# pangenome/povu

Hardware: AMD Instinct MI355X
Metric: edges/sec decomposed (flubble+PVST) (higher is better)
Workload: dtype u32

## Files before the change

### povu_amd/csrc/hip/common.hpp

```cpp
#pragma once
#include <hip/hip_runtime.h>

#include "forest_wire.hpp"

#include <algorithm>
#include <cstdint>
#include <cstdio>
#include <cstring>
#include <stdexcept>
#include <string>
#include <vector>

#define POVU_NIL 0xFFFFFFFFu

__device__ __forceinline__ uint4 load4_unaligned(const unsigned *__restrict__ p)
{
	typedef unsigned v4a __attribute__((ext_vector_type(4), aligned(4)));
	const v4a v = *reinterpret_cast<const v4a *>(p);
	return make_uint4(v.x, v.y, v.z, v.w);
}

#ifdef POVU_XCD_SWIZZLE
__device__ __forceinline__ unsigned povu_xcd_bid()
{
	const unsigned nwg = gridDim.x, q = nwg >> 3, r = nwg & 7u, x = blockIdx.x & 7u, i = blockIdx.x >> 3;
	return (x < r ? x * (q + 1) : r * (q + 1) + (x - r) * q) + i;
}
#define BIDX povu_xcd_bid()
#else
#define BIDX blockIdx.x
#endif

namespace povu_hip
{

struct HipError : std::runtime_error {
	using std::runtime_error::runtime_error;
};

#define HIP_CHECK(expr)                                                                          \
	do {                                                                                     \
		hipError_t e__ = (expr);                                                         \
		if (e__ != hipSuccess)                                                           \
			throw povu_hip::HipError(std::string(#expr) + ": " + hipGetErrorString(e__) + " (" + \
						 __FILE__ + ":" + std::to_string(__LINE__) + ")");   \
	} while (0)

#define KLAUNCH(kernel, grid, block, shmem, stream, ...)                                          \
	do {                                                                                      \
		hipLaunchKernelGGL(kernel, grid, block, shmem, stream, __VA_ARGS__);              \
		HIP_CHECK(hipGetLastError());                                                     \
	} while (0)
static constexpr int TPB = 256;
static inline unsigned nblk(size_t n) { return (unsigned)((n + TPB - 1) / TPB); }
#define LAUNCH(k, n, s, ...)                                                                     \
	do {                                                                                     \
		if ((n) > 0) {                                                                   \
			hipLaunchKernelGGL(k, dim3(nblk(n)), dim3(TPB), 0, s, __VA_ARGS__);      \
			HIP_CHECK(hipGetLastError());                                            \
		}                                                                                \
	} while (0)

struct XferTally {
	uint64_t h2d = 0, d2h = 0;
};
inline XferTally &xfer_tally()
{
	static thread_local XferTally t;
	return t;
}
inline hipError_t copy_async(void *dst, const void *src, size_t n, hipMemcpyKind kind, hipStream_t s)
{
	if (kind == hipMemcpyHostToDevice)
		xfer_tally().h2d += n;
	else if (kind == hipMemcpyDeviceToHost)
		xfer_tally().d2h += n;
	return hipMemcpyAsync(dst, src, n, kind, s);
}
inline void count_kernel_d2h(size_t n) { xfer_tally().d2h += n; }

class Arena
{
public:
	~Arena() { release(); }
	void release()
	{
		if (base_)
			(void)hipFree(base_);
		base_ = nullptr;
		cap_ = 0;
		top_ = 0;
	}
	void reserve(size_t bytes, bool head_room = true)
	{
		if (bytes > cap_) {
			release();
			size_t want = head_room ? bytes + bytes / 8 + (1u << 20) : bytes + 4096;
			if (hipMalloc(&base_, want) != hipSuccess) {
				(void)hipGetLastError();
				base_ = nullptr;
				want = bytes + 4096;
				if (hipMalloc(&base_, want) != hipSuccess) {
// ... 401 lines not shown
```

### povu_amd/csrc/hip/tree_kernels.hip

```cpp
#include "tree_kernels.hpp"

#include <cstdlib>

#include <algorithm>
#include <type_traits>
#include <vector>

namespace povu_hip
{

#ifndef NIL
#define NIL POVU_NIL
#endif

static unsigned rank_bucket_bits(size_t n)
{
	if (const char *ev = getenv("POVU_HIP_RANK_BITS"))
		return (unsigned)std::min(6, std::max(2, atoi(ev)));
	(void)n;
	return 3u;
}
static constexpr uint32_t PK_END = 0x1FFFFFFFu, PK_STOP = 0x80000000u;
static constexpr uint32_t P0_END = 0x3FFFFFFFu, P0_W = 0x40000000u, P0_HEAD = 0x80000000u;
static constexpr uint32_t FT_NONE = 0x7FFFFFFFu, FT_HASH = 0x80000000u;
__device__ __forceinline__ uint32_t bucket_splitter(uint32_t q, unsigned b) { return (q << b) | ((q * 0x9E3779B1u) >> (32u - b)); }
__device__ __forceinline__ bool is_splitter(uint32_t i, unsigned b) { return bucket_splitter(i >> b, b) == i; }
__device__ __forceinline__ uint32_t rank_pack(uint32_t nx, uint32_t w, unsigned b)
{
	(void)b;
	return (nx == NIL ? P0_END : nx) | ((w & 1u) ? P0_W : 0u);
}
__device__ __forceinline__ bool rank_l0_stop(uint32_t nx, unsigned b) { return nx == P0_END || is_splitter(nx, b); }

__device__ __forceinline__ uint32_t find_link_slot(const uint32_t *__restrict__ loff, const uint32_t *__restrict__ lle, uint32_t w,
						   uint32_t le)
{
	uint32_t lo = loff[w], hi = loff[w + 1];
	const uint32_t l0 = lo;
	if (hi - lo > 8) {
		while (lo < hi) {
			const uint32_t mid = (lo + hi) >> 1;
			if ((lle[mid] & LLE_ID) < le)
				lo = mid + 1;
			else
				hi = mid;
		}
		return lo - l0 + 1;
	}
	for (uint32_t j = lo; j < hi; j++)
		if ((lle[j] & LLE_ID) == le)
			return j - l0 + 1;
	return 0;
}
__device__ __forceinline__ void store2_unaligned(uint32_t *p, uint32_t a, uint32_t b)
{
	typedef uint32_t v2a __attribute__((ext_vector_type(2), aligned(4)));
	v2a v;
	v.x = a;
	v.y = b;
	*reinterpret_cast<v2a *>(p) = v;
}
__device__ __forceinline__ void zero2(uint32_t *p) { store2_unaligned(p, 0u, 0u); }
__device__ __forceinline__ void zero2(uint8_t *p) { p[0] = p[1] = 0; }
__device__ __forceinline__ uint32_t arc_twin(const uint32_t *__restrict__ loff, const uint32_t *__restrict__ ladj,
					     const uint32_t *__restrict__ lle, uint32_t at)
{
	const uint32_t w = ladj[at];
	return loff[w] + find_link_slot(loff, lle, w, lle[at] & LLE_ID) - 1;
}
__device__ __forceinline__ ulonglong2 link_hash(uint32_t le)
{
	unsigned long long z = ((unsigned long long)le + 1ull) * 0x9E3779B97F4A7C15ull;
	z = (z ^ (z >> 30)) * 0xBF58476D1CE4E5B9ull;
	z = (z ^ (z >> 27)) * 0x94D049BB133111EBull;
	unsigned long long y = ((unsigned long long)le ^ 0x5851F42D4C957F2Dull) * 0xD6E8FEB86659FD93ull;
	y = (y ^ (y >> 33)) * 0xFF51AFD7ED558CCDull;
	y = (y ^ (y >> 33)) * 0xC4CEB9FE1A85EC53ull;
	return make_ulonglong2(z ^ (z >> 31), y ^ (y >> 33));
}
__device__ __forceinline__ ulonglong2 hx(const ulonglong2 a, const ulonglong2 b) { return make_ulonglong2(a.x ^ b.x, a.y ^ b.y); }
__device__ __forceinline__ bool hzero(const ulonglong2 a) { return (a.x | a.y) == 0ull; }
__device__ __forceinline__ bool heq(const ulonglong2 a, const ulonglong2 b) { return a.x == b.x && a.y == b.y; }
__global__ void k_tour_words(uint32_t nS, const uint32_t *__restrict__ loff, const uint32_t *__restrict__ ladj,
			     const uint32_t *__restrict__ lle, uint32_t *__restrict__ pk, unsigned b,
			     ulonglong2 *__restrict__ hside, uint32_t *__restrict__ ft)
{
	uint32_t S = BIDX * blockDim.x + threadIdx.x;
	if (S >= nS)
		return;
	const uint32_t lo = loff[S], hi = loff[S + 1];
	ulonglong2 h = make_ulonglong2(0ull, 0ull);
	uint32_t first = NIL;
	for (uint32_t at0 = lo; at0 < hi; at0 += 4) {
		const uint32_t rem = hi - at0;
		const uint4 lw4 = load4_unaligned(lle + at0), w4 = load4_unaligned(ladj + at0);
		const uint32_t lws[4] = {lw4.x, lw4.y, lw4.z, lw4.w}, ws[4] = {w4.x, w4.y, w4.z, w4.w};
		bool tree[4];
		uint2 o01[4];
		uint32_t se[4];
#pragma unroll
		for (uint32_t q = 0; q < 4; q++) {
			tree[q] = q < rem && (lws[q] & LLE_TREE);
			o01[q] = make_uint2(0u, 0u);
			se[q] = 0;
			if (tree[q]) {
				const uint32_t g2 = ws[q] & ~1u;
				o01[q] = *reinterpret_cast<const uint2 *>(loff + g2);
				se[q] = loff[g2 + 2];
			}
		}
		uint4 a[4];
#pragma unroll
		for (uint32_t q = 0; q < 4; q++) {
			a[q] = make_uint4(0u, 0u, 0u, 0u);
			if (tree[q] && se[q] - o01[q].x <= 8)
				a[q] = load4_unaligned(lle + o01[q].x);
		}
#pragma unroll
		for (uint32_t q = 0; q < 4; q++) {
			if (q >= rem)
				break;
			const uint32_t at = at0 + q, lw = lws[q], le = lw & LLE_ID;
			if (!tree[q]) {
				pk[at] = P0_END;
				h = hx(h, link_hash(le));
				continue;
			}
			if (first == NIL)
				first = at;
			const uint32_t w = ws[q], sb = o01[q].x;
			const uint32_t wl = (w & 1u) ? o01[q].y : sb, wh = (w & 1u) ? se[q] : o01[q].y;
			uint32_t nxt;
			if (se[q] - sb <= 8) {
				const uint32_t n = se[q] - sb, tl = wl - sb, th = wh - sb;
				uint4 c = make_uint4(0u, 0u, 0u, 0u);
				if (n > 4)
					c = load4_unaligned(lle + sb + 4);
				const uint32_t r[8] = {a[q].x, a[q].y, a[q].z, a[q].w, c.x, c.y, c.z, c.w};
				uint32_t tk = 0, first_tree = NIL, after = NIL;
#pragma unroll
				for (uint32_t k = 0; k < 8; k++)
					if (k >= tl && k < th && (r[k] & LLE_ID) == le)
						tk = k;
#pragma unroll
				for (uint32_t k = 0; k < 8; k++)
					if (k < n && (r[k] & LLE_TREE)) {
						if (first_tree == NIL)
							first_tree = k;
						if (k > tk && after == NIL)
							after = k;
					}
				nxt = sb + (after != NIL ? after : (first_tree < tk ? first_tree : tk));
			} else {
				const uint32_t t = wl + find_link_slot(loff, lle, w, le) - 1;
				nxt = t;
				for (uint32_t jj = t + 1; jj < se[q] && nxt == t; jj++)
					if (lle[jj] & LLE_TREE)
						nxt = jj;
				for (uint32_t jj = sb; jj < t && nxt == t; jj++)
					if (lle[jj] & LLE_TREE)
						nxt = jj;
			}
			pk[at] = rank_pack(nxt, 1u, b);
		}
	}
	const bool nz = !hzero(h);
	if (nz)
		hside[S] = h;
	ft[S] = (first == NIL ? FT_NONE : first) | (nz ? FT_HASH : 0u);
}
__device__ __forceinline__ uint32_t comp_root_side(const unsigned long long *start_key, const uint32_t *voff, uint32_t c)
{
	unsigned long long k = start_key[c];
	return k == ~0ull ? 2 * voff[c] : (uint32_t)(k & 0xFFFFFFFFu);
}
__global__ void k_tour_ends(uint32_t C, const uint32_t *__restrict__ voff, const unsigned long long *__restrict__ start_key,
			    const uint32_t *__restrict__ loff, const uint32_t *__restrict__ ladj, const uint32_t *__restrict__ lle,
			    uint32_t *__restrict__ pk, uint32_t *__restrict__ heads)
{
	uint32_t c = BIDX * blockDim.x + threadIdx.x;
	if (c >= C)
		return;
	const uint32_t r = comp_root_side(start_key, voff, c), sb = loff[r & ~1u], se = loff[(r & ~1u) + 2], mid = loff[r];
	uint32_t a_first = NIL, a_last = NIL;
	for (uint32_t j = mid; j < se; j++)
		if (lle[j] & LLE_TREE) {
			if (a_first == NIL)
				a_first = j;
			a_last = j;
		}
	for (uint32_t j = sb; j < mid; j++)
		if (lle[j] & LLE_TREE) {
			if (a_first == NIL)
				a_first = j;
			a_last = j;
		}
	heads[c] = a_first;
	if (a_first == NIL)
		return;
	pk[arc_twin(loff, ladj, lle, a_last)] = P0_END;
// ... 159 lines not shown
		return;
	uint32_t sa = ra[id], sb = TWO ? rb[id] : 0, p;
	do {
		p = nx_in[x];
		const uint32_t wa = a_io[x];
		a_io[x] = sa;
		sa -= wa;
		if (TWO) {
			const uint32_t wb = b_io[x];
			b_io[x] = sb;
			sb -= wb;
		}
		x = p & PK_END;
	} while (!(p & PK_STOP));
}
template <bool TWO>
__global__ void __launch_bounds__(1024) k_rank_top(uint32_t n, const uint32_t *__restrict__ nx_in, uint32_t *a_io, uint32_t *b_io)
{
	__shared__ uint32_t nx[RANK_TOP], sa[RANK_TOP], sb[TWO ? RANK_TOP : 1];
	for (uint32_t i = threadIdx.x; i < n; i += blockDim.x) {
		const uint32_t p = nx_in[i] & PK_END;
		nx[i] = p == PK_END ? NIL : p;
		sa[i] = a_io[i];
		if (TWO)
			sb[i] = b_io[i];
	}
	__syncthreads();
	constexpr int PER = RANK_TOP / 1024;
	for (uint32_t span = 1; span < n; span <<= 1) {
		uint32_t tn[PER], ta[PER], tb[PER];
#pragma unroll
		for (int k = 0; k < PER; k++) {
			const uint32_t i = threadIdx.x + k * 1024;
			tn[k] = NIL, ta[k] = 0, tb[k] = 0;
			if (i < n && nx[i] != NIL) {
				const uint32_t j = nx[i];
				tn[k] = nx[j];
				ta[k] = sa[j];
				if (TWO)
					tb[k] = sb[j];
			}
		}
		__syncthreads();
#pragma unroll
		for (int k = 0; k < PER; k++) {
			const uint32_t i = threadIdx.x + k * 1024;
			if (i < n && nx[i] != NIL) {
				nx[i] = tn[k];
				sa[i] += ta[k];
				if (TWO)
					sb[i] += tb[k];
			}
		}
		__syncthreads();
	}
	for (uint32_t i = threadIdx.x; i < n; i += blockDim.x) {
		a_io[i] = sa[i];
		if (TWO)
			b_io[i] = sb[i];
	}
}
__global__ void k_rank_unpack_next(uint32_t n, const uint32_t *__restrict__ nx_in, uint32_t *__restrict__ out)
{
	uint32_t i = BIDX * blockDim.x + threadIdx.x;
	if (i < n) {
		const uint32_t p = nx_in[i] & PK_END;
		out[i] = p == PK_END ? NIL : p;
	}
}

struct RankBufs {
	uint32_t *pk;
	uint32_t *heads;
	uint32_t *nx, *wa, *wb;
	uint32_t *tA, *tB, *tC;
};
static constexpr int RANK_MAX_LEVELS = 12;
static size_t rank_pool_words(size_t n, size_t nh) { return n / 2 + 4 * nh + 64; }

struct L0Ranks {
	const uint32_t *ra, *rb, *fin;
	uint32_t M;
};
__device__ __forceinline__ uint32_t rank_l0(const L0Ranks &R, uint2 rec)
{
	return (rec.x < R.M ? R.ra[rec.x] : 0u) - rec.y;
}
__device__ __forceinline__ uint32_t rank_l0_a(const L0Ranks &R, uint2 rec, bool fin)
{
	return fin ? rec.x : (rec.x < R.M ? R.ra[rec.x] : 0u) - (rec.y & REC_MAX);
}
__device__ __forceinline__ uint2 rank_l0_pair(const L0Ranks &R, uint2 rec, bool fin)
{
	if (fin)
		return rec;
	const bool in = rec.x < R.M;
	const uint32_t ra = in ? R.ra[rec.x] : 0u, rb = in ? R.rb[rec.x] : 0u, pa = rec.y & REC_MAX;
	return make_uint2(ra - pa, rb - pa + (rec.y >> 16));
}

template <bool TWO, bool EVT3 = false>
static L0Ranks list_rank_splitters(uint32_t n, unsigned b, uint2 *rec, uint32_t *ovf, uint32_t nh, RankBufs &rb, hipStream_t s)
{
	if (n >= P0_END)
		throw HipError("list ranking: more than 2^30 elements (graph too large for the packed walk)");
	RankLevelArgs lv[RANK_MAX_LEVELS];
	uint32_t *nxp[RANK_MAX_LEVELS + 1], *wap[RANK_MAX_LEVELS + 1], *wbp[RANK_MAX_LEVELS + 1];
	int levels = 0;
	size_t used = 0;
	const size_t pool = rank_pool_words(n, nh);
	nxp[0] = rb.pk, wap[0] = wbp[0] = nullptr;
	uint32_t cur_n = n, hbase = 0;
	for (;;) {
		RankLevelArgs &A = lv[levels];
		A.n = cur_n;
		A.m = (cur_n + (1u << b) - 1) >> b;
		A.hbase = hbase;
		A.M = A.m + nh;
		if (used + A.M > pool)
			throw HipError("list ranking: level pool exhausted (internal sizing bug)");
		nxp[levels + 1] = rb.nx + used, wap[levels + 1] = rb.wa + used, wbp[levels + 1] = rb.wb + used;
		used += A.M;
		levels++;
		hbase = A.m;
		const uint32_t next_n = A.M;
		if (next_n <= RANK_TOP || next_n > cur_n / 2 || levels == RANK_MAX_LEVELS) {
			cur_n = next_n;
			break;
		}
		cur_n = next_n;
	}
	if (TWO)
		HIP_CHECK(hipMemsetAsync(ovf, 0, 4, s));
	for (int L = 0; L < levels; L++) {
		const RankLevelArgs &A = lv[L];
		if (L == 0)
			LAUNCH((k_rank_up<true, TWO, EVT3>), A.M, s, A, b, nxp[0], nullptr, nullptr, rb.heads, nxp[1], wap[1], wbp[1], rec, ovf);
		else
			LAUNCH((k_rank_up<false, TWO>), A.M, s, A, b, nxp[L], wap[L], wbp[L], nullptr, nxp[L + 1], wap[L + 1], wbp[L + 1],
			       nullptr, nullptr);
	}
	const uint32_t nt = cur_n;
	if (nt <= RANK_TOP) {
		KLAUNCH((k_rank_top<TWO>), dim3(1), dim3(1024), 0, s, nt, nxp[levels], wap[levels], wbp[levels]);
	} else {
		LAUNCH(k_rank_unpack_next, nt, s, nt, nxp[levels], rb.tA);
		HIP_CHECK(copy_async(rb.tB, wap[levels], (size_t)nt * 4, hipMemcpyDeviceToDevice, s));
		if (TWO)
			HIP_CHECK(copy_async(rb.tC, wbp[levels], (size_t)nt * 4, hipMemcpyDeviceToDevice, s));
		uint32_t *nA = rb.tA, *nB = nxp[levels], *aA = rb.tB, *aB = wap[levels], *bA = rb.tC, *bB = wbp[levels];
		const int side = list_rank(nt, bits_for(nt) + 1, nA, nB, aA, aB, TWO ? bA : nullptr, TWO ? bB : nullptr, s);
		if (side == 0) {
			HIP_CHECK(copy_async(wap[levels], aA, (size_t)nt * 4, hipMemcpyDeviceToDevice, s));
			if (TWO)
				HIP_CHECK(copy_async(wbp[levels], bA, (size_t)nt * 4, hipMemcpyDeviceToDevice, s));
		}
	}
	for (int L = levels - 1; L >= 1; L--) {
		const RankLevelArgs &A = lv[L];
		LAUNCH((k_rank_down<TWO>), A.M, s, A, b, nxp[L], wap[L], wbp[L], wap[L + 1], wbp[L + 1]);
	}
	if (TWO)
		KLAUNCH((k_rank_l0_fallback<EVT3>), dim3(std::min(nblk(lv[0].M), 2048u)), dim3(TPB), 0, s, lv[0], b, rb.pk, rb.heads, wap[1],
			wbp[1], rec, ovf);
	return L0Ranks{wap[1], TWO ? wbp[1] : nullptr, TWO ? ovf : nullptr, lv[0].M};
}

template <bool TWO>
__global__ void k_rank_resolve(uint32_t n, const uint2 *__restrict__ rec, L0Ranks R, uint32_t *__restrict__ ra, uint32_t *__restrict__ rb)
{
	const uint32_t x = BIDX * blockDim.x + threadIdx.x;
	if (x >= n)
		return;
	if (TWO) {
		const uint2 r = rank_l0_pair(R, rec[x], *R.fin != 0);
		ra[x] = r.x;
		rb[x] = r.y;
	} else {
		ra[x] = rank_l0(R, rec[x]);
	}
}
void debug_list_rank(uint32_t n, const uint32_t *next, const uint8_t *w, const uint32_t *heads, uint32_t nh, int mode,
		     unsigned bits, uint32_t *ra, uint32_t *rb, hipStream_t s)
{
	if (n == 0 || n >= P0_END)
		throw HipError("debug_list_rank: n must be in [1, 2^30)");
	const unsigned b = bits ? std::min(6u, std::max(2u, bits)) : rank_bucket_bits(n);
	std::vector<uint32_t> pk(n);
	for (uint32_t x = 0; x < n; x++) {
		if (next[x] != NIL && next[x] >= n)
			throw HipError("debug_list_rank: successor out of range");
		pk[x] = (next[x] == NIL ? P0_END : next[x]) | (w[x] ? P0_W : 0u);
	}
	for (uint32_t h = 0; h < nh; h++)
		if (heads[h] != NIL) {
			if (heads[h] >= n)
				throw HipError("debug_list_rank: head out of range");
			pk[heads[h]] |= P0_HEAD;
		}
	const size_t pool = rank_pool_words(n, nh);
	Arena ar;
	ar.reserve(Arena::padded(n + 16, 4) * 3 + Arena::padded(n + 16, 8) + Arena::padded(nh + 1, 4) + 6 * Arena::padded(pool, 4) + 8192, false);
	RankBufs rbf{};
	rbf.pk = ar.take<uint32_t>(n + 16);
	rbf.heads = ar.take<uint32_t>(nh + 1);
	for (uint32_t **q : {&rbf.nx, &rbf.wa, &rbf.wb, &rbf.tA, &rbf.tB, &rbf.tC})
		*q = ar.take<uint32_t>(pool);
	uint32_t *da = ar.take<uint32_t>(n + 16), *db = ar.take<uint32_t>(n + 16), *ovf = ar.take<uint32_t>(4);
	uint2 *rec = ar.take<uint2>(n + 16);
	HIP_CHECK(copy_async(rbf.pk, pk.data(), (size_t)n * 4, hipMemcpyHostToDevice, s));
	if (nh)
		HIP_CHECK(copy_async(rbf.heads, heads, (size_t)nh * 4, hipMemcpyHostToDevice, s));
	if (mode == 0) {
		const L0Ranks R = list_rank_splitters<false>(n, b, rec, nullptr, nh, rbf, s);
		LAUNCH(k_rank_resolve<false>, n, s, n, rec, R, da, nullptr);
	} else {
		const L0Ranks R = list_rank_splitters<true, true>(n, b, rec, ovf, nh, rbf, s);
		LAUNCH(k_rank_resolve<true>, n, s, n, rec, R, da, db);
	}
	HIP_CHECK(copy_async(ra, da, (size_t)n * 4, hipMemcpyDeviceToHost, s));
	if (mode != 0)
		HIP_CHECK(copy_async(rb, db, (size_t)n * 4, hipMemcpyDeviceToHost, s));
	HIP_CHECK(hipStreamSynchronize(s));
}

static constexpr uint32_t T0_RBIT = 0x80000000u;
static constexpr uint32_t BS_POS = 0x3FFFFFFFu, BS_NOARC = 0x80000000u, BS_HASH_L = 0x40000000u, BS_HASH_R = 0x80000000u;
__global__ void k_t0_parents(uint32_t V, const uint2 *__restrict__ trec, L0Ranks R, const uint32_t *__restrict__ ckey,
			     const uint32_t *__restrict__ voff, const uint32_t *__restrict__ loff, const uint32_t *__restrict__ ladj,
			     const uint32_t *__restrict__ lle,
			     const uint32_t *__restrict__ ft, const uint32_t *__restrict__ heads,
			     uint4 *__restrict__ t0seg, uint2 *__restrict__ fstr, uint4 *__restrict__ xrec, uint32_t C,
			     const unsigned long long *__restrict__ start_key, uint32_t *__restrict__ err, uint8_t *__restrict__ multi)
{
	uint32_t g = BIDX * blockDim.x + threadIdx.x;
	if (g < V)
		*reinterpret_cast<uint16_t *>(multi + 2 * g) = 0;
	if (g < C) {
		const uint32_t r = comp_root_side(start_key, voff, g), L = 2 * (voff[g + 1] - voff[g] - 1);
		t0seg[r >> 1] = make_uint4(NIL, (r & 1u) ? T0_RBIT : 0u, 0u, L ? L - 1 : 0u);
		const uint32_t h = heads[g];
		if (h == NIL ? L != 0 : rank_l0(R, trec[h]) != L - 1)
			atomicExch(err, 1u);
	}
	if (g >= V)
		return;
	const uint32_t sb = loff[2 * g], sm = loff[2 * g + 1], se = loff[2 * g + 2];
	const uint2 f2 = *reinterpret_cast<const uint2 *>(ft + 2 * g);
	uint32_t at_e = NIL, dmin = 0xFFFFFFFFu, dmax = 0u;
	uint32_t a_l = NIL, a_r = NIL, d_l = 0u, d_r = 0u;
	for (uint32_t at0 = sb; at0 < se; at0 += 4) {
		const uint32_t *r32 = reinterpret_cast<const uint32_t *>(trec + at0);
		const uint4 lw4 = load4_unaligned(lle + at0), r01 = load4_unaligned(r32), r23 = load4_unaligned(r32 + 4);
		const uint32_t lws[4] = {lw4.x, lw4.y, lw4.z, lw4.w};
		const uint2 rs[4] = {make_uint2(r01.x, r01.y), make_uint2(r01.z, r01.w), make_uint2(r23.x, r23.y), make_uint2(r23.z, r23.w)};
		bool tree[4];
		uint32_t ds[4];
#pragma unroll
		for (uint32_t q = 0; q < 4; q++) {
			tree[q] = at0 + q < se && (lws[q] & LLE_TREE);
			ds[q] = tree[q] ? rank_l0(R, rs[q]) : 0u;
		}
#pragma unroll
		for (uint32_t q = 0; q < 4; q++) {
			if (!tree[q])
				continue;
			if (ds[q] < dmin) {
				dmin = ds[q];
				at_e = at0 + q;
			}
			dmax = max(dmax, ds[q]);
			if (at0 + q < sm) {
				if (a_l == NIL)
					a_l = at0 + q, d_l = ds[q];
			} else if (a_r == NIL) {
				a_r = at0 + q, d_r = ds[q];
			}
		}
	}
	const uint32_t hbits = ((f2.x & FT_HASH) ? BS_HASH_L : 0u) | ((f2.y & FT_HASH) ? BS_HASH_R : 0u);
	if (at_e == NIL) {
		fstr[g] = make_uint2(BS_NOARC, hbits);
		return;
	}
	const uint32_t c = ckey[g], root = comp_root_side(start_key, voff, c);
	const uint32_t L = 2 * (voff[c + 1] - voff[c] - 1), abase = 2 * (voff[c] - c);
	if ((root >> 1) == g) {
		const bool far_r = !(root & 1u);
		const uint32_t a1 = far_r ? a_r : a_l, d1 = far_r ? d_r : d_l;
		fstr[g] = a1 == NIL ? make_uint2(BS_NOARC, hbits) : make_uint2((abase + (L - 1 - d1)) & BS_POS, ((abase + L) & BS_POS) | hbits);
		return;
	}
	const uint32_t p_in = abase + (L - 2 - dmax), p_out = abase + (L - 1 - dmin);
	t0seg[g] = make_uint4(ladj[at_e], (lle[at_e] & LLE_ID) | (at_e >= sm ? T0_RBIT : 0u), p_in, p_out);
	{
		const bool ent_r = at_e >= sm;
		const uint32_t a1 = ent_r ? a_l : a_r, d1 = ent_r ? d_l : d_r, a3 = ent_r ? a_r : a_l, d3 = ent_r ? d_r : d_l;
		const uint32_t end = a3 != at_e ? abase + (L - 1 - d3) : p_out;
		fstr[g] = a1 == NIL ? make_uint2(BS_NOARC, hbits) : make_uint2((abase + (L - 1 - d1)) & BS_POS, (end & BS_POS) | hbits);
	}
	if ((f2.x | f2.y) & FT_HASH)
		atomicOr(reinterpret_cast<unsigned long long *>(&xrec[p_in >> 6]), 1ull << (p_in & 63u));
}
__global__ void k_tour_values(uint32_t V, const uint4 *__restrict__ t0seg, const uint32_t *__restrict__ ft,
			      const ulonglong2 *__restrict__ hside, const uint4 *__restrict__ xrec, ulonglong2 *__restrict__ xval)
{
	uint32_t g = BIDX * blockDim.x + threadIdx.x;
	if (g >= V)
		return;
	const uint2 f2 = *reinterpret_cast<const uint2 *>(ft + 2 * g);
	if (!((f2.x | f2.y) & FT_HASH))
		return;
	const uint4 r = t0seg[g];
	if (r.x == NIL)
		return;
	const ulonglong2 z = make_ulonglong2(0ull, 0ull);
	xval[bitrank(xrec, r.z)] = hx((f2.x & FT_HASH) ? hside[2 * g] : z, (f2.y & FT_HASH) ? hside[2 * g + 1] : z);
}
static constexpr uint32_t PB_BRIDGE = 0x80000000u;
static constexpr uint32_t CLASS_BUDGET = 256;
static constexpr uint32_t CS_VISITED = 0x40000000u;
__global__ void k_bridges(uint32_t V, const uint4 *__restrict__ t0seg, const uint2 *__restrict__ fstr,
			  const ulonglong2 *__restrict__ xps, const uint4 *__restrict__ xrec,
			  const ulonglong2 *__restrict__ hside, const uint32_t *__restrict__ loff, const uint32_t *__restrict__ lle,
			  const uint32_t *__restrict__ ckey, const uint32_t *__restrict__ cproc,
			  uint8_t *multi, uint32_t *__restrict__ cstate, uint2 *__restrict__ dps)
{
	const uint32_t g = BIDX * blockDim.x + threadIdx.x;
	if (g >= V)
		return;
	auto stretch = [&](uint32_t p, uint32_t q) {
		const uint32_t rp = bitrank(xrec, p), rq = bitrank(xrec, q);
		return rp == rq ? make_ulonglong2(0ull, 0ull) : hx(xps[rp], xps[rq]);
	};
	const uint4 r = t0seg[g];
	const uint32_t Se = (2 * g) | (r.y >> 31), Sf = Se ^ 1u, c = ckey[g];
	const bool proc = cproc[c] != 0;
	uint32_t pvE;
	if (r.x == NIL) {
		pvE = NIL;
	} else if (hzero(stretch(r.z, r.w + 1))) {
		pvE = r.x | PB_BRIDGE;
	} else {
		pvE = r.x;
		multi[Se] = 1;
// ... 49 lines not shown
		const uint32_t S0 = B0 + it * (TPB * 4u) + threadIdx.x * 4u;
		uint32_t f = 0;
		if (S0 + 4 <= nS) {
			const uint4 pb = *reinterpret_cast<const uint4 *>(pbr + S0);
			const uint32_t mu = *reinterpret_cast<const uint32_t *>(multi + S0);
			const uint2 ck = *reinterpret_cast<const uint2 *>(ckey + (S0 >> 1));
			const uint32_t c0 = cproc[ck.x] ? 1u : 0u, c1 = cproc[ck.y] ? 1u : 0u;
			f = (((mu & 0xFFu) && (pb.x & PB_BRIDGE)) ? c0 : 0u) | ((((mu & 0xFF00u) && (pb.y & PB_BRIDGE)) ? c0 : 0u) << 1) |
			    ((((mu & 0xFF0000u) && (pb.z & PB_BRIDGE)) ? c1 : 0u) << 2) | ((((mu & 0xFF000000u) && (pb.w & PB_BRIDGE)) ? c1 : 0u) << 3);
		} else {
			for (uint32_t S = S0; S < nS; S++)
				f |= ((multi[S] && (pbr[S] & PB_BRIDGE) && cproc[ckey[S >> 1]]) ? 1u : 0u) << (S - S0);
		}
		fw |= (unsigned long long)f << (4 * it);
	}
	append_in_order(fw, B0, entry_list, n_entry);
}

static constexpr uint32_t W_UNVIS = 0xFFFFFFFEu;
static constexpr uint32_t W_INLINE = 6;
static constexpr uint32_t W_CHUNK0 = 64;
struct WalkRec {
	uint32_t n, begin, c[W_INLINE];
};
__global__ void k_class_recs(uint32_t nS, const uint32_t *__restrict__ loff, const uint32_t *__restrict__ ladj,
			     const uint32_t *__restrict__ pbr, const uint32_t *__restrict__ ckey,
			     const uint32_t *__restrict__ cproc, uint32_t *__restrict__ wadj, uint4 *__restrict__ wrec,
			     uint32_t *__restrict__ wpar)
{
	uint32_t u = BIDX * blockDim.x + threadIdx.x;
	if (u >= nS)
		return;
	const uint32_t lo = loff[u], hi = loff[u + 1], base = lo + u;
	uint32_t n = 0, c[W_INLINE] = {NIL, NIL, NIL, NIL, NIL, NIL};
	uint32_t vis = W_UNVIS;
	if (cproc[ckey[u >> 1]]) {
		const uint32_t mine = pbr[u] & ~CS_VISITED;
		if (mine & PB_BRIDGE)
			vis = 0u;
		auto same_class = [&](uint32_t o) { return o != u && mine != (o | PB_BRIDGE) && (pbr[o] & ~CS_VISITED) != (u | PB_BRIDGE); };
		auto put = [&](uint32_t o) {
			if (n < W_INLINE) {
#pragma unroll
				for (uint32_t k = 0; k < W_INLINE; k++)
					if (k == n)
						c[k] = o;
			} else {
				if (n == W_INLINE)
					for (uint32_t k = 0; k < W_INLINE; k++)
						wadj[base + k] = c[k];
				wadj[base + n] = o;
			}
			n++;
		};
		if (same_class(u ^ 1u))
			put(u ^ 1u);
		for (uint32_t k = lo; k < hi; k++) {
			const uint32_t o = ladj[k];
			if (same_class(o))
				put(o);
		}
	}
	wrec[2 * (size_t)u] = make_uint4(n, base, c[0], c[1]);
	wrec[2 * (size_t)u + 1] = make_uint4(c[2], c[3], c[4], c[5]);
	wpar[u] = vis;
}
static constexpr uint32_t DFS_STK = 8;
__global__ void __launch_bounds__(64) k_class_dfs_small(const uint32_t *__restrict__ n_entry_dev, const uint32_t *__restrict__ entry_list,
							 const uint32_t *__restrict__ loff, const uint32_t *__restrict__ ladj,
							 uint32_t *__restrict__ cstate, uint2 *__restrict__ dps, uint32_t budget,
							 uint32_t *__restrict__ n_over, uint32_t *__restrict__ over_list)
{
	__shared__ uint4 stk[DFS_STK][64];
	const uint32_t lane = threadIdx.x;
	const uint32_t n_entry = *n_entry_dev;
	for (uint32_t i = BIDX * blockDim.x + threadIdx.x; i < n_entry; i += gridDim.x * blockDim.x) {
		const uint32_t s = entry_list[i];
		const uint32_t s_up = cstate[s] & ~(CS_VISITED | PB_BRIDGE);
		uint32_t u = s, k = 0, lo = loff[u], n = loff[u + 1] - lo, sides = 0, depth = 0;
		for (;;) {
			bool adv = false;
			while (k <= n) {
				const uint32_t rem = n + 1 - k;
				uint32_t o0, o1, o2, o3;
				if (k == 0) {
					const uint4 x = load4_unaligned(ladj + lo);
					o0 = u ^ 1u, o1 = x.x, o2 = x.y, o3 = x.z;
				} else {
					const uint4 x = load4_unaligned(ladj + lo + k - 1);
					o0 = x.x, o1 = x.y, o2 = x.z, o3 = x.w;
				}
				const uint32_t w0 = cstate[o0];
				const uint32_t w1 = rem > 1 ? cstate[o1] : CS_VISITED;
				const uint32_t w2 = rem > 2 ? cstate[o2] : CS_VISITED;
				const uint32_t w3 = rem > 3 ? cstate[o3] : CS_VISITED;
				auto open = [&](uint32_t o, uint32_t w) { return !(w & CS_VISITED) && !(u == s && o == s_up); };
				const uint32_t j = open(o0, w0) ? 0u : open(o1, w1) ? 1u : open(o2, w2) ? 2u : open(o3, w3) ? 3u : 4u;
				if (j == 4) {
					k += min(rem, 4u);
					continue;
				}
				const uint32_t o = j == 0 ? o0 : j == 1 ? o1 : j == 2 ? o2 : o3, w = j == 0 ? w0 : j == 1 ? w1 : j == 2 ? w2 : w3;
				const uint32_t slot = k + j;
				k = slot + 1;
				const uint32_t g2 = o & ~1u, odd = o & 1u;
				uint32_t l0, l1, l2 = 0, wp = CS_VISITED;
				if (slot == 0) {
					l0 = loff[o], l1 = loff[o + 1];
				} else {
					const uint4 l4 = load4_unaligned(loff + g2);
					l0 = l4.x, l1 = l4.y, l2 = l4.z;
					const uint2 cs2 = *reinterpret_cast<const uint2 *>(cstate + g2);
					wp = odd ? cs2.x : cs2.y;
				}
				const uint32_t nlo = (slot == 0 || !odd) ? l0 : l1, nhi = (slot == 0) ? l1 : (odd ? l2 : l1);
				if (depth < DFS_STK)
					stk[depth][lane] = make_uint4(u, k, lo, n);
				depth++;
				sides++;
				if (!(wp & CS_VISITED)) {
					const uint32_t p = o ^ 1u, plo = odd ? l0 : l1, phi = odd ? l1 : l2;
					const uint32_t so = w | CS_VISITED, sp = wp | CS_VISITED;
					*reinterpret_cast<uint2 *>(cstate + g2) = odd ? make_uint2(sp, so) : make_uint2(so, sp);
					*reinterpret_cast<uint4 *>(dps + g2) = odd ? make_uint4(o, 0u, u, slot) : make_uint4(u, slot, o, 0u);
					if (depth < DFS_STK)
						stk[depth][lane] = make_uint4(o, 1u, nlo, nhi - nlo);
					depth++;
					sides++;
					u = p;
					lo = plo;
					n = phi - plo;
				} else {
					cstate[o] = w | CS_VISITED;
					dps[o] = make_uint2(u, slot);
					u = o;
					lo = nlo;
					n = nhi - nlo;
				}
				k = 1;
				adv = true;
				break;
			}
			if (adv) {
				if (sides > budget) {
					over_list[atomicAdd(n_over, 1u)] = s;
					break;
				}
				continue;
			}
			if (u == s)
				break;
			depth--;
			if (depth < DFS_STK) {
				const uint4 r = stk[depth][lane];
				u = r.x, k = r.y, lo = r.z, n = r.w;
			} else {
				const uint2 up = dps[u];
				k = up.y + 1;
				u = up.x;
				lo = loff[u];
				n = loff[u + 1] - lo;
			}
		}
	}
}
struct WalkStackEntry {
	uint32_t u, j;
	uint4 r0, r1;
};
__device__ __forceinline__ uint32_t wstk_addr(uint32_t d, const uint32_t *chunk_base)
{
	const uint32_t c = d < W_CHUNK0 ? 0u : 32u - (uint32_t)__clz(d / W_CHUNK0);
	return chunk_base[c] + (d - (c ? (W_CHUNK0 << (c - 1)) : 0u));
}
__device__ __forceinline__ uint32_t wrec_cand(const uint4 &r0, const uint4 &r1, uint32_t k)
{
	return k == 0 ? r0.z : k == 1 ? r0.w : k == 2 ? r1.x : k == 3 ? r1.y : k == 4 ? r1.z : r1.w;
}
static constexpr uint32_t W_WIN = 128;
static constexpr uint32_t W_WIN_BACK = 16;
__device__ __forceinline__ uint32_t sgpr(uint32_t v) { return __builtin_amdgcn_readfirstlane(v); }
__device__ __forceinline__ uint32_t lane_val(uint32_t v, int l) { return __builtin_amdgcn_readlane(v, l); }
struct URec {
	uint32_t n, begin, c0, c1, c2, c3, c4, c5;
};
__device__ __forceinline__ URec urec_lane(const uint4 a, const uint4 b, int l)
{
	return URec{lane_val(a.x, l), lane_val(a.y, l), lane_val(a.z, l), lane_val(a.w, l),
		    lane_val(b.x, l), lane_val(b.y, l), lane_val(b.z, l), lane_val(b.w, l)};
}
template <bool HOT>
__global__ void __launch_bounds__(64) k_class_walk_wave(uint32_t n_entry, const uint32_t *__restrict__ entry_list,
							 const uint4 *__restrict__ wrec, const uint32_t *__restrict__ wadj,
							 uint32_t *wpar, uint2 *wstk, uint32_t *__restrict__ pool_top, uint32_t pool_cap,
							 uint32_t *__restrict__ err, uint32_t nS, uint32_t route)
{
	__shared__ uint4 win_rec[W_WIN][2];
	__shared__ uint32_t win_par[W_WIN];
// ... 219 lines not shown
	}
	uint32_t enter = rank_pack(c_o != NIL ? 3 * (c_o >> 1) : A + 1, 0u, b);
	if (p == NIL) {
		const uint32_t comp = ckey[g];
		if (cproc[comp]) {
			enter |= P0_HEAD;
			heads[comp] = A;
		}
	}
	pk[A] = enter;
	if (ns_o != NIL) {
		pk[A + 1] = rank_pack(3 * (ns_o >> 1), 0u, b);
		pk[A + 2] = rank_pack(after_e, 0u, b);
		merged[g] = 0;
	} else {
		pk[A + 1] = rank_pack(after_e, 1u, b);
		pk[A + 2] = P0_END;
		merged[g] = 1;
	}
}

template <typename OC, typename SC, typename IC>
__global__ void k_tree_emit(uint32_t nS, const uint2 *__restrict__ erec, L0Ranks R, const uint8_t *__restrict__ merged,
			    const uint2 *__restrict__ dps, const uint32_t *__restrict__ ckey,
			    const uint32_t *__restrict__ cproc, const uint32_t *__restrict__ voff,
			    const unsigned long long *__restrict__ start_key, const uint32_t *__restrict__ gid_s,
			    uint32_t *__restrict__ t_gid, uint8_t *__restrict__ t_flags, uint32_t *__restrict__ t_par,
			    uint32_t *__restrict__ t_size, uint32_t *__restrict__ t_depth, uint32_t *__restrict__ side_tidx,
			    uint32_t C, uint32_t *__restrict__ c_ntree, OC *__restrict__ ordcnt, uint32_t *__restrict__ hi0,
			    uint32_t *__restrict__ mpre, SC *__restrict__ srccnt, uint32_t *__restrict__ sdl,
			    IC *__restrict__ incnt)
{
	uint32_t S = BIDX * blockDim.x + threadIdx.x;
	if (S == 0) {
		const uint32_t T = 2 * (nS >> 1) + C;
		hi0[T] = NIL;
		srccnt[T] = srccnt[T + 1] = 0;
		incnt[T] = incnt[T + 1] = 0;
	}
	if (S < C) {
		const uint32_t Nr = 2 * (voff[S + 1] - voff[S]), tr = 2 * voff[S] + S;
		if (!cproc[S]) {
			c_ntree[S] = 0;
			t_size[tr + Nr] = 0;
			srccnt[tr + Nr] = 0;
			incnt[tr + Nr] = 0;
		} else {
			const uint32_t hr = start_key[S] != ~0ull ? 1u : 0u;
			c_ntree[S] = Nr + hr;
			if (hr) {
				t_gid[tr] = NIL;
				t_flags[tr] = 2 | TF_ROOT;
				t_par[tr] = NIL;
				t_size[tr] = Nr + 1;
				incnt[tr] = 0;
				if (t_depth)
					t_depth[tr] = 0;
				mpre[tr] = tr;
				ordcnt[tr] = 0;
				hi0[tr] = NIL;
			} else {
				t_size[tr + Nr] = 0;
				srccnt[tr + Nr] = 0;
				incnt[tr + Nr] = 0;
			}
		}
	}
	const uint32_t g = S;
	if (g >= (nS >> 1))
		return;
	const uint32_t c = ckey[g], v0 = voff[c];
	const uint32_t tb = 2 * v0 + c;
	if (!cproc[c]) {
		const uint32_t t = tb + 2 * (g - v0);
		store2_unaligned(t_size + t, 0u, 0u);
		zero2(srccnt + t);
		zero2(incnt + t);
		*reinterpret_cast<uint2 *>(side_tidx + 2 * g) = make_uint2(NIL, NIL);
		return;
	}
	const uint32_t Nh = 2 * (voff[c + 1] - v0), hd = start_key[c] != ~0ull ? 1u : 0u;
	const bool fin = *R.fin != 0;
	const uint4 r01 = load4_unaligned(reinterpret_cast<const uint32_t *>(erec + 3 * g));
	const uint2 ent = rank_l0_pair(R, make_uint2(r01.x, r01.y), fin);
	const uint2 lv_o = make_uint2(rank_l0_a(R, make_uint2(r01.z, r01.w), fin), 0u);
	const uint4 d4 = *reinterpret_cast<const uint4 *>(dps + 2 * g);
	const uint32_t o = d4.x == 2 * g + 1 ? 2 * g : 2 * g + 1, e = o ^ 1u;
	const uint32_t p = (e & 1u) ? d4.z : d4.x;
	const uint32_t pre_e = Nh - ent.x, depth_e = 0u - ent.y;
	uint32_t lv_e = lv_o.x;
	if (!merged[g]) {
		lv_e = rank_l0_a(R, erec[3 * g + 2], fin);
	}
	const uint32_t size_o = ent.x - 1 - lv_o.x, size_e = ent.x - lv_e;
	uint32_t par_e;
	if (p == NIL)
		par_e = hd ? 0u : NIL;
	else {
		par_e = hd + (Nh - rank_l0_a(R, erec[3 * (p >> 1)], fin)) + (dps[p].x == (p ^ 1u) ? 1u : 0u);
	}
	const uint32_t l = hd + pre_e, t = tb + l;
	const uint32_t gid = gid_s[g];
	store2_unaligned(t_gid + t, gid, gid);
	t_flags[t] = (uint8_t)((e & 1u) | (par_e == NIL ? TF_ROOT : 0u));
	t_flags[t + 1] = (uint8_t)((o & 1u) | TF_BLACK);
	store2_unaligned(t_par + t, par_e, l);
	store2_unaligned(t_size + t, size_e, size_o);
	zero2(incnt + t);
	if (t_depth)
		store2_unaligned(t_depth + t, depth_e + hd, depth_e + 1 + hd);
	store2_unaligned(mpre + t, tb + (depth_e + hd) + (Nh + hd) - l - size_e, tb + (depth_e + 1 + hd) + (Nh + hd) - (l + 1) - size_o);
	*reinterpret_cast<uint2 *>(side_tidx + 2 * g) = (e & 1u) ? make_uint2(t + 1, t) : make_uint2(t, t + 1);
	if (sdl) {
		const uint32_t gray = (size_e - 1 - size_o) / 2, black = (size_o + 1) / 2, gs = v0 + pre_e / 2;
		if (gray) {
			atomicAdd(&sdl[gs], gray);
			atomicAdd(&sdl[gs + black], 0u - gray - black);
			atomicAdd(&sdl[gs + size_e / 2], black);
		}
	}
}
#ifndef POVU_BE_ITER
#define POVU_BE_ITER 8
#endif
static constexpr uint32_t BE_ITER = POVU_BE_ITER, BE_SIDES = TPB * BE_ITER;
template <bool EMIT, typename IC>
__device__ __forceinline__ uint32_t side_back_edges(uint32_t S, uint32_t p, uint32_t at,
						    const uint32_t *__restrict__ loff, const uint32_t *__restrict__ ladj,
						    const uint2 *__restrict__ dps, const uint32_t *__restrict__ side_tidx,
						    const uint32_t *__restrict__ ckey, const uint32_t *__restrict__ voff,
						    const uint32_t *__restrict__ t_par, uint32_t *__restrict__ b_src,
						    uint32_t *__restrict__ b_tgt, uint32_t *__restrict__ b_ord,
						    const uint8_t *__restrict__ dupflag, IC *__restrict__ incnt, uint32_t &highest,
						    uint32_t *first2)
{
	uint32_t n = 0;
	const uint32_t c = ckey[S >> 1], root = 2 * voff[c] + c;
	const uint32_t lo = loff[S], hi = loff[S + 1];
	auto out = [&](uint32_t tgt) {
		if (EMIT) {
			b_src[at + n] = p;
			b_tgt[at + n] = tgt;
			b_ord[at + n] = n;
			if (sizeof(IC) == 4 || tgt != root)
				incnt_add(incnt, tgt);
		} else {
			highest = min(highest, tgt);
			if (n < 2)
				first2[n] = tgt;
		}
		n++;
	};
	if (lo == hi) {
		if (p == root || t_par[p] != 0)
			out(root);
		return n;
	}
	const uint32_t dp = dps[S].x;
	bool loop_seen = false;
	for (uint32_t k0 = lo; k0 < hi; k0 += 4) {
		const uint4 o4 = load4_unaligned(ladj + k0);
		const uint32_t rem = hi - k0;
		const uint32_t os[4] = {o4.x, o4.y, o4.z, o4.w};
		const uint32_t xs[4] = {side_tidx[o4.x], rem > 1 ? side_tidx[o4.y] : NIL, rem > 2 ? side_tidx[o4.z] : NIL,
					rem > 3 ? side_tidx[o4.w] : NIL};
#pragma unroll
		for (uint32_t q = 0; q < 4; q++) {
			if (q >= rem)
				break;
			const uint32_t k = k0 + q, o = os[q], x = xs[q];
			if (o == (S ^ 1)) {
				if (dp == o && !loop_seen)
					out(x);
				loop_seen = true;
				continue;
			}
			if (x > p || o == dp)
				continue;
			bool dup = false;
			if (dupflag) {
				dup = dupflag[k] != 0;
			} else {
				for (uint32_t j = lo; j < k; j++)
// ... 542 lines not shown
```

Baseline: 3.247 billion.

## Make gathers unconditional with safe indices and batch them before use

Replaces conditional loads in several tree kernels with predicated-index gathers that always issue, pointing at a safe in-bounds address when the condition is false. Empty inline-asm barriers ("landed") group the loads so they are all in flight before any result is consumed. The aim is more memory-level parallelism and less divergent control flow, so dependent gather latencies overlap instead of running one after another. In exchange every lane issues extra loads, which raises memory traffic, and the asm constraints may tie down registers and limit scheduling freedom.

```diff
diff --git a/povu_amd/csrc/hip/common.hpp b/povu_amd/csrc/hip/common.hpp
--- a/povu_amd/csrc/hip/common.hpp
+++ b/povu_amd/csrc/hip/common.hpp
@@ -18,6 +18,35 @@
 	typedef unsigned v4a __attribute__((ext_vector_type(4), aligned(4)));
 	const v4a v = *reinterpret_cast<const v4a *>(p);
 	return make_uint4(v.x, v.y, v.z, v.w);
+}
+
+#define POVU_W2(v) "+v"((v).x), "+v"((v).y)
+#define POVU_W4(v) "+v"((v).x), "+v"((v).y), "+v"((v).z), "+v"((v).w)
+__device__ __forceinline__ void landed(uint32_t &a, uint32_t &b, uint32_t &c, uint32_t &d) { asm volatile("" : "+v"(a), "+v"(b), "+v"(c), "+v"(d)); }
+__device__ __forceinline__ void landed(uint32_t &a, uint32_t &b, uint32_t &c, uint32_t &d, uint32_t &e)
+{
+	asm volatile("" : "+v"(a), "+v"(b), "+v"(c), "+v"(d), "+v"(e));
+}
+__device__ __forceinline__ void landed(uint2 &a, uint2 &b, uint2 &c, uint2 &d, uint32_t &e, uint32_t &f, uint32_t &g, uint32_t &h)
+{
+	asm volatile("" : POVU_W2(a), POVU_W2(b), POVU_W2(c), POVU_W2(d), "+v"(e), "+v"(f), "+v"(g), "+v"(h));
+}
+__device__ __forceinline__ void landed(uint4 &a, uint2 &b) { asm volatile("" : POVU_W4(a), POVU_W2(b)); }
+__device__ __forceinline__ void landed(uint4 &a, uint4 &b, uint4 &c, uint4 &d) { asm volatile("" : POVU_W4(a), POVU_W4(b), POVU_W4(c), POVU_W4(d)); }
+#undef POVU_W2
+#undef POVU_W4
+template <class T>
+__device__ __forceinline__ T gather_if(bool cond, const T *__restrict__ p, uint32_t i, uint32_t safe)
+{
+	return p[cond ? i : safe];
+}
+__device__ __forceinline__ uint2 gather2_if(bool cond, const unsigned *__restrict__ p, uint32_t i, uint32_t safe)
+{
+	return *reinterpret_cast<const uint2 *>(p + (cond ? i : safe));
+}
+__device__ __forceinline__ uint4 gather4_unaligned_if(bool cond, const unsigned *__restrict__ p, uint32_t i, uint32_t safe)
+{
+	return load4_unaligned(p + (cond ? i : safe));
 }
 
 #ifdef POVU_XCD_SWIZZLE
diff --git a/povu_amd/csrc/hip/tree_kernels.hip b/povu_amd/csrc/hip/tree_kernels.hip
--- a/povu_amd/csrc/hip/tree_kernels.hip
+++ b/povu_amd/csrc/hip/tree_kernels.hip
@@ -101,21 +101,17 @@
 #pragma unroll
 		for (uint32_t q = 0; q < 4; q++) {
 			tree[q] = q < rem && (lws[q] & LLE_TREE);
-			o01[q] = make_uint2(0u, 0u);
-			se[q] = 0;
-			if (tree[q]) {
-				const uint32_t g2 = ws[q] & ~1u;
-				o01[q] = *reinterpret_cast<const uint2 *>(loff + g2);
-				se[q] = loff[g2 + 2];
-			}
-		}
+			o01[q] = gather2_if(tree[q], loff, ws[q] & ~1u, S & ~1u);
+			se[q] = gather_if(tree[q], loff, (ws[q] & ~1u) + 2, (S & ~1u) + 2);
+		}
+		landed(o01[0], o01[1], o01[2], o01[3], se[0], se[1], se[2], se[3]);
 		uint4 a[4];
 #pragma unroll
 		for (uint32_t q = 0; q < 4; q++) {
-			a[q] = make_uint4(0u, 0u, 0u, 0u);
-			if (tree[q] && se[q] - o01[q].x <= 8)
-				a[q] = load4_unaligned(lle + o01[q].x);
-		}
+			const uint32_t n = se[q] - o01[q].x;
+			a[q] = gather4_unaligned_if(tree[q] && n <= 8, lle, o01[q].x, at0);
+		}
+		landed(a[0], a[1], a[2], a[3]);
 #pragma unroll
 		for (uint32_t q = 0; q < 4; q++) {
 			if (q >= rem)
@@ -441,21 +437,23 @@
 	const uint32_t *ra, *rb, *fin;
 	uint32_t M;
 };
-__device__ __forceinline__ uint32_t rank_l0(const L0Ranks &R, uint2 rec)
-{
-	return (rec.x < R.M ? R.ra[rec.x] : 0u) - rec.y;
-}
-__device__ __forceinline__ uint32_t rank_l0_a(const L0Ranks &R, uint2 rec, bool fin)
-{
-	return fin ? rec.x : (rec.x < R.M ? R.ra[rec.x] : 0u) - (rec.y & REC_MAX);
-}
+__device__ __forceinline__ uint32_t l0_at(const L0Ranks &R, uint2 rec, bool want = true) { return want && rec.x < R.M ? rec.x : 0u; }
+__device__ __forceinline__ uint32_t rank_l0(const L0Ranks &R, uint2 rec, uint32_t ra) { return (rec.x < R.M ? ra : 0u) - rec.y; }
+__device__ __forceinline__ uint32_t rank_l0_a(const L0Ranks &R, uint2 rec, bool fin, uint32_t ra)
+{
+	return fin ? rec.x : (rec.x < R.M ? ra : 0u) - (rec.y & REC_MAX);
+}
+__device__ __forceinline__ uint2 rank_l0_pair(const L0Ranks &R, uint2 rec, bool fin, uint32_t ra, uint32_t rb)
+{
+	const bool in = rec.x < R.M;
+	const uint32_t pa = rec.y & REC_MAX;
+	return fin ? rec : make_uint2((in ? ra : 0u) - pa, (in ? rb : 0u) - pa + (rec.y >> 16));
+}
+__device__ __forceinline__ uint32_t rank_l0(const L0Ranks &R, uint2 rec) { return rank_l0(R, rec, R.ra[l0_at(R, rec)]); }
 __device__ __forceinline__ uint2 rank_l0_pair(const L0Ranks &R, uint2 rec, bool fin)
 {
-	if (fin)
-		return rec;
-	const bool in = rec.x < R.M;
-	const uint32_t ra = in ? R.ra[rec.x] : 0u, rb = in ? R.rb[rec.x] : 0u, pa = rec.y & REC_MAX;
-	return make_uint2(ra - pa, rb - pa + (rec.y >> 16));
+	const uint32_t i = l0_at(R, rec, !fin);
+	return rank_l0_pair(R, rec, fin, R.ra[i], R.rb[i]);
 }
 
 template <bool TWO, bool EVT3 = false>
@@ -618,8 +616,12 @@
 #pragma unroll
 		for (uint32_t q = 0; q < 4; q++) {
 			tree[q] = at0 + q < se && (lws[q] & LLE_TREE);
-			ds[q] = tree[q] ? rank_l0(R, rs[q]) : 0u;
-		}
+			ds[q] = R.ra[l0_at(R, rs[q], tree[q])];
+		}
+		landed(ds[0], ds[1], ds[2], ds[3]);
+#pragma unroll
+		for (uint32_t q = 0; q < 4; q++)
+			ds[q] = rank_l0(R, rs[q], ds[q]);
 #pragma unroll
 		for (uint32_t q = 0; q < 4; q++) {
 			if (!tree[q])
@@ -835,18 +837,11 @@
 			bool adv = false;
 			while (k <= n) {
 				const uint32_t rem = n + 1 - k;
-				uint32_t o0, o1, o2, o3;
-				if (k == 0) {
-					const uint4 x = load4_unaligned(ladj + lo);
-					o0 = u ^ 1u, o1 = x.x, o2 = x.y, o3 = x.z;
-				} else {
-					const uint4 x = load4_unaligned(ladj + lo + k - 1);
-					o0 = x.x, o1 = x.y, o2 = x.z, o3 = x.w;
-				}
-				const uint32_t w0 = cstate[o0];
-				const uint32_t w1 = rem > 1 ? cstate[o1] : CS_VISITED;
-				const uint32_t w2 = rem > 2 ? cstate[o2] : CS_VISITED;
-				const uint32_t w3 = rem > 3 ? cstate[o3] : CS_VISITED;
+				const uint4 x = load4_unaligned(ladj + lo + (k ? k - 1 : 0u));
+				const uint32_t o0 = k ? x.x : u ^ 1u, o1 = k ? x.y : x.x, o2 = k ? x.z : x.y, o3 = k ? x.w : x.z;
+				uint32_t w0 = cstate[o0], w1 = gather_if(rem > 1, cstate, o1, 0u), w2 = gather_if(rem > 2, cstate, o2, 0u), w3 = gather_if(rem > 3, cstate, o3, 0u);
+				landed(w0, w1, w2, w3);
+				w1 = rem > 1 ? w1 : CS_VISITED, w2 = rem > 2 ? w2 : CS_VISITED, w3 = rem > 3 ? w3 : CS_VISITED;
 				auto open = [&](uint32_t o, uint32_t w) { return !(w & CS_VISITED) && !(u == s && o == s_up); };
 				const uint32_t j = open(o0, w0) ? 0u : open(o1, w1) ? 1u : open(o2, w2) ? 2u : open(o3, w3) ? 3u : 4u;
 				if (j == 4) {
@@ -857,16 +852,12 @@
 				const uint32_t slot = k + j;
 				k = slot + 1;
 				const uint32_t g2 = o & ~1u, odd = o & 1u;
-				uint32_t l0, l1, l2 = 0, wp = CS_VISITED;
-				if (slot == 0) {
-					l0 = loff[o], l1 = loff[o + 1];
-				} else {
-					const uint4 l4 = load4_unaligned(loff + g2);
-					l0 = l4.x, l1 = l4.y, l2 = l4.z;
-					const uint2 cs2 = *reinterpret_cast<const uint2 *>(cstate + g2);
-					wp = odd ? cs2.x : cs2.y;
-				}
-				const uint32_t nlo = (slot == 0 || !odd) ? l0 : l1, nhi = (slot == 0) ? l1 : (odd ? l2 : l1);
+				uint4 l4 = load4_unaligned(loff + g2);
+				uint2 cs2 = *reinterpret_cast<const uint2 *>(cstate + (slot ? g2 : 0u));
+				landed(l4, cs2);
+				const uint32_t l0 = l4.x, l1 = l4.y, l2 = l4.z;
+				const uint32_t wp = slot == 0 ? CS_VISITED : (odd ? cs2.x : cs2.y);
+				const uint32_t nlo = odd ? l1 : l0, nhi = odd ? l2 : l1;
 				if (depth < DFS_STK)
 					stk[depth][lane] = make_uint4(u, k, lo, n);
 				depth++;
@@ -1252,23 +1243,28 @@
 	const uint32_t Nh = 2 * (voff[c + 1] - v0), hd = start_key[c] != ~0ull ? 1u : 0u;
 	const bool fin = *R.fin != 0;
 	const uint4 r01 = load4_unaligned(reinterpret_cast<const uint32_t *>(erec + 3 * g));
-	const uint2 ent = rank_l0_pair(R, make_uint2(r01.x, r01.y), fin);
-	const uint2 lv_o = make_uint2(rank_l0_a(R, make_uint2(r01.z, r01.w), fin), 0u);
+	const uint2 r2 = erec[3 * g + 2];
+	const bool two_leaves = !merged[g];
 	const uint4 d4 = *reinterpret_cast<const uint4 *>(dps + 2 * g);
 	const uint32_t o = d4.x == 2 * g + 1 ? 2 * g : 2 * g + 1, e = o ^ 1u;
 	const uint32_t p = (e & 1u) ? d4.z : d4.x;
+	const bool has_p = p != NIL;
+	const uint32_t pp = has_p ? p : e;
+	const uint2 r_p = erec[3 * (pp >> 1)], d_p = dps[pp];
+	const uint2 r0 = make_uint2(r01.x, r01.y), r1 = make_uint2(r01.z, r01.w);
+	const uint32_t i0 = l0_at(R, r0, !fin);
+	uint32_t a0 = R.ra[i0], b0 = R.rb[i0], a1 = R.ra[l0_at(R, r1, !fin)], a2 = R.ra[l0_at(R, r2, !fin && two_leaves)], a_p = R.ra[l0_at(R, r_p, !fin && has_p)];
+	landed(a0, b0, a1, a2, a_p);
+	const uint2 ent = rank_l0_pair(R, r0, fin, a0, b0), lv_o = make_uint2(rank_l0_a(R, r1, fin, a1), 0u);
+	const uint32_t lv_e2 = rank_l0_a(R, r2, fin, a2), ent_p = rank_l0_a(R, r_p, fin, a_p);
 	const uint32_t pre_e = Nh - ent.x, depth_e = 0u - ent.y;
-	uint32_t lv_e = lv_o.x;
-	if (!merged[g]) {
-		lv_e = rank_l0_a(R, erec[3 * g + 2], fin);
-	}
+	const uint32_t lv_e = two_leaves ? lv_e2 : lv_o.x;
 	const uint32_t size_o = ent.x - 1 - lv_o.x, size_e = ent.x - lv_e;
 	uint32_t par_e;
-	if (p == NIL)
+	if (!has_p)
 		par_e = hd ? 0u : NIL;
-	else {
-		par_e = hd + (Nh - rank_l0_a(R, erec[3 * (p >> 1)], fin)) + (dps[p].x == (p ^ 1u) ? 1u : 0u);
-	}
+	else
+		par_e = hd + (Nh - ent_p) + (d_p.x == (p ^ 1u) ? 1u : 0u);
 	const uint32_t l = hd + pre_e, t = tb + l;
 	const uint32_t gid = gid_s[g];
 	store2_unaligned(t_gid + t, gid, gid);
```

Measured after the change: 3.285 billion (median of 6 runs). +1.2%, better.
